# tbennun/capital

Hardware: NVIDIA H100
Metric: cholesky_tflops_fp64 (higher is better)
Workload: dtype f64

## Files before the change

capital_b200/csrc/api.cu:

```cuda
#include "common.cuh"
#include "dist.cuh"
#include "peer.cuh"
#include <math.h>
#include <stdlib.h>
#include <algorithm>

capital_status_t capital_ctx::workspace(const std::string& name, size_t bytes, void** out) {
  capital_ctx* ctx = this;
  DeviceBuf& b = pool[name];
  if (b.bytes < bytes) {
    if (b.p) CAP_CUDA(cudaFree(b.p));
    b.p = nullptr; b.bytes = 0;
    CAP_CUDA(cudaMalloc(&b.p, bytes));
    b.bytes = bytes;
    if (poison_workspace) {
      CAP_CUDA(cudaMemsetAsync(b.p, 0xFF, bytes, cudaStreamLegacy));
      CAP_CUDA(cudaStreamSynchronize(cudaStreamLegacy));
    }
  }
  *out = b.p;
  return CAPITAL_OK;
}

int capital_ctx::stream_id(cudaStream_t st) const {
// ... 368 lines not shown
capital_status_t capital_last_factor_ms(const capital_ctx* ctx_, float* ms) {
  capital_ctx* ctx = const_cast<capital_ctx*>(ctx_);
  if (!ctx || !ms) return CAPITAL_ERR_INVALID;
  CAP_CUDA(cudaEventElapsedTime(ms, ctx->ev_start, ctx->ev_stop));
  return CAPITAL_OK;
}

capital_status_t capital_timeline_begin(capital_ctx* ctx) {
  if (!ctx) return CAPITAL_ERR_INVALID;
  ctx->timeline = true; ctx->tl.clear(); ctx->tl_used = 0;
  return CAPITAL_OK;
}
capital_status_t capital_timeline_end(capital_ctx* ctx, double* out, int64_t cap_records, int64_t* n_records) {
  if (!ctx || !n_records) return CAPITAL_ERR_INVALID;
  ctx->timeline = false;
  CAP_CUDA(cudaSetDevice(ctx->device));
  CAP_CUDA(cudaDeviceSynchronize());
  *n_records = (int64_t)ctx->tl.size();
  if (out && !ctx->tl.empty()) {
    cudaEvent_t base = ctx->tl[0].e0;
    for (auto& r : ctx->tl) {
      float d = 0;
      if (cudaEventElapsedTime(&d, base, r.e0) == cudaSuccess && d < 0) base = r.e0;
    }
    for (int64_t i = 0; i < *n_records && i < cap_records; i++) {
      const auto& r = ctx->tl[i];
      float t0 = 0, t1 = 0;
      CAP_CUDA(cudaEventElapsedTime(&t0, base, r.e0));
      CAP_CUDA(cudaEventElapsedTime(&t1, base, r.e1));
      double* o = out + i * 8;
      o[0] = r.sid; o[1] = r.kind; o[2] = t0; o[3] = t1; o[4] = r.a; o[5] = r.b; o[6] = r.c; o[7] = 0;
    }
  }
  return CAPITAL_OK;
}
capital_status_t capital_probe_dmma_f64(capital_ctx* ctx, double* tflops, double* ms) {
  if (!ctx || !tflops || !ms) return CAPITAL_ERR_INVALID;
  CAP_CUDA(cudaSetDevice(ctx->device));
  return gemm_probe_dmma(ctx, tflops, ms);
}
capital_status_t capital_set_overlap(capital_ctx* ctx, int enabled) {
  if (!ctx) return CAPITAL_ERR_INVALID;
  ctx->no_overlap = !enabled;
  return CAPITAL_OK;
}
capital_status_t capital_profile_begin(capital_ctx* ctx) {
  if (!ctx) return CAPITAL_ERR_INVALID;
  ctx->profiling = true; ctx->prof_used = 0; ctx->prof_recs.clear();
  return CAPITAL_OK;
}
capital_status_t capital_profile_end(capital_ctx* ctx, double* kernel_ms, double* kernel_flops, int64_t* launches) {
  if (!ctx || !kernel_ms || !kernel_flops || !launches) return CAPITAL_ERR_INVALID;
  ctx->profiling = false;
  CAP_CUDA(cudaStreamSynchronize(ctx->stream));
  double ms = 0, fl = 0;
  for (auto& r : ctx->prof_recs) {
    float t = 0;
    CAP_CUDA(cudaEventElapsedTime(&t, r.e0, r.e1));
    ms += t; fl += r.flops;
  }
  *kernel_ms = ms; *kernel_flops = fl; *launches = (int64_t)ctx->prof_recs.size();
  ctx->prof_recs.clear(); ctx->prof_used = 0;
  return CAPITAL_OK;
}

capital_status_t capital_distribute_symmetric_f64(capital_ctx* ctx, double* A_local, int64_t n, int diag_dom) {
  if (!ctx || !A_local || n <= 0) return CAPITAL_ERR_INVALID;
  CAP_CUDA(cudaSetDevice(ctx->device));
  const int d = ctx->grid.d;
  const int64_t L = ceil_div(n, d);
  double* dev;
  CAP_TRY(cap_stage_out_begin(ctx, A_local, (size_t)L * L, "gen_out", &dev));
  CAP_TRY(gen_symmetric(ctx, ctx->stream, dev, L, L, L, n, ctx->grid.x, ctx->grid.y, d, diag_dom));
  CAP_TRY(cap_stage_out_end(ctx, A_local, (size_t)L * L, dev));
  CAP_CUDA(cudaStreamSynchronize(ctx->stream));
  return CAPITAL_OK;
}
capital_status_t capital_distribute_random_f64(capital_ctx* ctx, double* A_local, int64_t m, int64_t n, int64_t key) {
  if (!ctx || !A_local || n <= 0 || m <= 0) return CAPITAL_ERR_INVALID;
  CAP_CUDA(cudaSetDevice(ctx->device));
  const int c = ctx->grid.c, d = ctx->grid.d, x = ctx->grid.x, y = ctx->grid.y;
  const int64_t lr = ceil_div(m, d), lc = ceil_div(n, c);
  const int64_t pad_c = ((n % c != 0) && ((lc - 1) * c + x >= n)) ? lc - 1 : lc;
  const int64_t pad_r = ((m % d != 0) && ((lr - 1) * d + y >= m)) ? lr - 1 : lr;
  double* dev;
  CAP_TRY(cap_stage_out_begin(ctx, A_local, (size_t)lr * lc, "gen_out", &dev));
  CAP_TRY(gen_random(ctx, ctx->stream, dev, lr, lr, lc, pad_r, pad_c, key));
  CAP_TRY(cap_stage_out_end(ctx, A_local, (size_t)lr * lc, dev));
  CAP_CUDA(cudaStreamSynchronize(ctx->stream));
  return CAPITAL_OK;
}

capital_status_t capital_cholinv_factor_f64(capital_ctx* ctx, const double* A_local, int64_t n, const capital_cholinv_args_t* args,
                                            capital_structure_t ostruct, double* R_local, double* Rinv_local) {
  if (!ctx) return CAPITAL_ERR_INVALID;
  if (!A_local || !args || !R_local || !Rinv_local || n <= 0 || args->split <= 0 || args->dir != 'U') {
    ctx->set_error("cholinv::factor: invalid arguments (split > 0 and dir == 'U' are required, cholinv.hpp:9)");
    return CAPITAL_ERR_INVALID;
  }
  CAP_CUDA(cudaSetDevice(ctx->device));
  const capital_grid_t& g = ctx->grid;
  if (g.size > 1) return dist_cholinv_factor(ctx, A_local, n, args, ostruct, R_local, Rinv_local);

  const int64_t L = n, ld = round_up(L, 16);
  const size_t out_count = ostruct == CAPITAL_UPPERTRI_PACKED ? (size_t)L * (L + 1) / 2 : (size_t)L * L;
  cudaStream_t st = ctx->stream;
  ctx->io_used = 0;
  CAP_CUDA(cudaEventRecord(ctx->ev_start, st));
  double *W, *Rm, *Ri, *RiT, *dR, *dRinv;
  CAP_TRY(ctx->workspace("W", (size_t)ld * L * 8, (void**)&W));
  CAP_TRY(ctx->workspace("Rm", (size_t)ld * L * 8, (void**)&Rm));
  CAP_TRY(ctx->workspace("Ri", (size_t)ld * L * 8, (void**)&Ri));
  CAP_TRY(ctx->workspace("RiT", (size_t)ld * L * 8, (void**)&RiT));
  CAP_TRY(cap_stage_out_begin(ctx, R_local, out_count, "R_out", &dR));
  CAP_TRY(cap_stage_out_begin(ctx, Rinv_local, out_count, "Rinv_out", &dRinv));
  CAP_CUDA(cudaMemsetAsync(ctx->d_info, 0, sizeof(int), st));
  const int64_t bc = capital_cholinv_bc_dimension(L, g.c, g.d, args->bc_mult_dim);
  if (ostruct == CAPITAL_RECT) {
    CAP_CUDA(cudaMemsetAsync(Ri, 0, (size_t)ld * L * 8, st));
  } else {
    CAP_TRY(zero_band(ctx, st, L, Ri, ld));
    if (args->complete_inv == 0 && cholinv_node_splits(L, bc, (int)args->split)) {
      const int64_t s1 = L >> args->split;
      if (s1 > 0 && s1 < L) CAP_TRY(zero_block(ctx, st, s1, L - s1, Ri + s1 * ld, ld));
    }
  }
  CAP_TRY(zero_band(ctx, st, L, RiT, ld));
  if (ostruct == CAPITAL_RECT) CAP_CUDA(cudaMemsetAsync(Rm, 0, (size_t)ld * L * 8, st));

  HostIO io;
  io.ctx = ctx; io.L = L; io.ld = ld; io.Rm = Rm; io.Ri = Ri; io.dR = dR; io.dRinv = dRinv;
  io.hR = (dR != R_local) ? R_local : nullptr; io.hRinv = (dRinv != Rinv_local) ? Rinv_local : nullptr;
  io.packed = ostruct == CAPITAL_UPPERTRI_PACKED;
  io.rinv_streams = args->complete_inv == 0 && cholinv_node_splits(L, bc, (int)args->split);
  CholinvHooks hooks{&io, nullptr, nullptr};
  if (!cap_is_device_ptr(A_local)) {
    cudaEvent_t e0;
    CAP_TRY(io_event(ctx, &e0));
    CAP_CUDA(cudaEventRecord(e0, st));
    CAP_CUDA(cudaStreamWaitEvent(ctx->copy_in, e0, 0));
    const int64_t chunk = round_up(ceil_div(L, 16), 64);
    for (int64_t c0 = 0; c0 < L; c0 += chunk) {
      const int64_t nc = (c0 + chunk <= L) ? chunk : L - c0;
      const int64_t rows = c0 + nc;
      CAP_CUDA(cudaMemcpy2DAsync(W + c0 * ld, (size_t)ld * 8, A_local + c0 * L, (size_t)L * 8, (size_t)rows * 8, (size_t)nc,
                                 cudaMemcpyHostToDevice, ctx->copy_in));
      ctx->counters.h2d_bytes += rows * nc * 8;
      cudaEvent_t e;
      CAP_TRY(io_event(ctx, &e));
      CAP_CUDA(cudaEventRecord(e, ctx->copy_in));
      io.chunks.push_back({c0 + nc, e});
    }
    hooks.need_cols = hostio_need_cols;
  } else {
    CAP_TRY(copy_block(ctx, st, L, L, A_local, L, W, ld));
  }
  if (io.packed && L >= 2048) hooks.left_done = hostio_left_done;
  if (hooks.need_cols) hooks.cols_waited = hostio_cols_waited;
  if (hooks.left_done && (io.hR || io.hRinv)) {
    hooks.right_done = hostio_right_done;
    if (io.hRinv) hooks.inv_cols = hostio_inv_cols;
  }
  CAP_TRY(cholinv_local(ctx, st, L, W, ld, Rm, ld, Ri, ld, RiT, ld, args->complete_inv != 0, bc, (int)args->split, &hooks));
  if (ostruct == CAPITAL_UPPERTRI_PACKED) {
    {
      const int64_t c0 = io.cols_out;
      const size_t off = (size_t)c0 * (c0 + 1) / 2, cnt = out_count - off;
      CAP_TRY(pack_upper(ctx, st, L, Rm, ld, dR, 0, c0, L));
      if (io.hR && cnt) { CAP_CUDA(cudaMemcpyAsync(io.hR + off, dR + off, cnt * 8, cudaMemcpyDeviceToHost, st)); ctx->counters.d2h_bytes += (int64_t)cnt * 8; }
    }
    {
      const int64_t c0 = io.rinv_cols_out;
      const size_t off = (size_t)c0 * (c0 + 1) / 2, cnt = out_count - off;
      CAP_TRY(pack_upper(ctx, st, L, Ri, ld, dRinv, 0, c0, L));
      if (io.hRinv && cnt) { CAP_CUDA(cudaMemcpyAsync(io.hRinv + off, dRinv + off, cnt * 8, cudaMemcpyDeviceToHost, st)); ctx->counters.d2h_bytes += (int64_t)cnt * 8; }
    }
    if (io.e_out) CAP_CUDA(cudaStreamWaitEvent(st, io.e_out, 0));
  } else {
    CAP_TRY(triu_copy(ctx, st, L, Rm, ld, dR, L, 0));
    CAP_TRY(triu_copy(ctx, st, L, Ri, ld, dRinv, L, 0));
    CAP_TRY(cap_stage_out_end(ctx, R_local, out_count, dR));
    CAP_TRY(cap_stage_out_end(ctx, Rinv_local, out_count, dRinv));
  }
  CAP_CUDA(cudaEventRecord(ctx->ev_stop, st));
  return cap_check_info(ctx);
}

capital_status_t capital_cholinv_residual_f64(capital_ctx* ctx, const double* A_local, int64_t n, capital_structure_t structure,
                                              const double* R_local, double* residual) {
  if (!ctx || !A_local || !R_local || !residual || n <= 0) return CAPITAL_ERR_INVALID;
  CAP_CUDA(cudaSetDevice(ctx->device));
  const capital_grid_t& g = ctx->grid;
  if (g.size > 1) return dist_cholinv_residual(ctx, A_local, n, structure, R_local, residual);
  const int64_t L = n, ld = round_up(L, 16);
  cudaStream_t st = ctx->stream;
  const size_t r_count = structure == CAPITAL_UPPERTRI_PACKED ? (size_t)L * (L + 1) / 2 : (size_t)L * L;
  const double *dA, *dRin;
  CAP_TRY(cap_stage_in(ctx, A_local, (size_t)L * L, "A_in", &dA));
  CAP_TRY(cap_stage_in(ctx, R_local, r_count, "R_in", &dRin));
  double *E, *Rr;
  CAP_TRY(ctx->workspace("W", (size_t)ld * L * 8, (void**)&E));
  CAP_TRY(ctx->workspace("Rm", (size_t)ld * L * 8, (void**)&Rr));
  if (structure == CAPITAL_UPPERTRI_PACKED) CAP_TRY(unpack_upper(ctx, st, L, dRin, Rr, ld));
  else CAP_TRY(triu_copy(ctx, st, L, dRin, L, Rr, ld, 0));
  CAP_TRY(copy_block(ctx, st, L, L, dA, L, E, ld));
  CAP_CUDA(cudaMemsetAsync(ctx->d_scalars, 0, 2 * sizeof(double), st));
  CAP_TRY(sumsq_block(ctx, st, L, L, E, ld, 1, 0, 0, 1, ctx->d_scalars + 1));
  CAP_TRY(gemm_tn(ctx, st, L, L, L, 1.0, Rr, ld, Rr, ld, -1.0, E, ld,
                  CAPITAL_GEMM_A_UPPER | CAPITAL_GEMM_B_UPPER | CAPITAL_GEMM_C_UPPER));
  CAP_TRY(sumsq_block(ctx, st, L, L, E, ld, 1, 0, 0, 1, ctx->d_scalars));
  double h[2];
  CAP_CUDA(cudaMemcpyAsync(h, ctx->d_scalars, 2 * sizeof(double), cudaMemcpyDeviceToHost, st));
  CAP_CUDA(cudaStreamSynchronize(st));
  *residual = sqrt(h[0]) / sqrt(h[1]);
  return CAPITAL_OK;
}

static capital_status_t cholinv_solve_mode(capital_ctx* ctx, int64_t n, const capital_cholinv_args_t* args, capital_structure_t structure,
                                           const double* R_local, const double* Rinv_local, int64_t nrhs, const double* B, int64_t ldb,
                                           double* X, int64_t ldx, int mode, const char* what) {
  const bool apply_r = mode == SOLVE_R || mode == SOLVE_RT;
  if (!args || (apply_r ? !R_local : !Rinv_local) || !B || !X || n <= 0 || nrhs < 1 || ldb < n || ldx < n || args->split <= 0 ||
      args->dir != 'U' || (structure != CAPITAL_RECT && structure != CAPITAL_UPPERTRI_PACKED)) {
    ctx->set_error(std::string("cholinv::") + what + ": invalid arguments (" + (apply_r ? "R" : "Rinv") +
                   ", B, X non-null, nrhs >= 1, ldb, ldx >= n, split > 0 and dir == 'U')");
    return CAPITAL_ERR_INVALID;
  }
  CAP_CUDA(cudaSetDevice(ctx->device));
  const capital_grid_t& g = ctx->grid;
  if (g.size > 1) return dist_cholinv_solve(ctx, n, args, structure, R_local, Rinv_local, nrhs, B, ldb, X, ldx, mode);
  const int64_t L = n;
  const int64_t bc = capital_cholinv_bc_dimension(L, g.c, g.d, args->bc_mult_dim);
  const bool skipped = !apply_r && args->complete_inv == 0 && cholinv_node_splits(L, bc, (int)args->split);
  if (skipped && !R_local) {
    ctx->set_error(std::string("cholinv::") + what + ": the top-level Rinv12 block was skipped (complete_inv = 0), R is needed");
    return CAPITAL_ERR_INVALID;
  }
  const int64_t s1 = L >> args->split;
  const bool packed = structure == CAPITAL_UPPERTRI_PACKED;
  const size_t f_count = packed ? (size_t)L * (L + 1) / 2 : (size_t)L * L;
  const int64_t ldu = packed ? 0 : L;
  cudaStream_t st = ctx->stream;
  const double *dRi = nullptr, *dR = nullptr, *dB;
  if (!apply_r) CAP_TRY(cap_stage_in(ctx, Rinv_local, f_count, "solve_Rinv", &dRi));
  if (skipped || apply_r) CAP_TRY(cap_stage_in(ctx, R_local, f_count, "solve_R", &dR));
  CAP_TRY(cap_stage_in(ctx, B, (size_t)ldb * (nrhs - 1) + n, "solve_B", &dB));
  const bool x_host = !cap_is_device_ptr(X);
  double* dX = X;
  if (x_host) CAP_TRY(ctx->workspace("solve_X", (size_t)ldx * nrhs * 8, (void**)&dX));
  double *T, *T2;
  CAP_TRY(ctx->workspace("solve_T", (size_t)L * SOLVE_W * 8, (void**)&T));
  CAP_TRY(ctx->workspace("solve_T2", (size_t)L * SOLVE_W * 8, (void**)&T2));
  auto half_t = [&](const double* Bp, int64_t w) -> capital_status_t {
    if (!skipped) return tri_apply(ctx, st, {dRi, ldu, true, 0, L, 0, L, w, 1.0, Bp, 1, ldb, 0.0, nullptr, 0, T, 1, L});
    CAP_TRY(tri_apply(ctx, st, {dRi, ldu, true, 0, s1, 0, s1, w, 1.0, Bp, 1, ldb, 0.0, nullptr, 0, T, 1, L}));
    CAP_TRY(tri_apply(ctx, st, {dR, ldu, true, 0, s1, s1, L, w, -1.0, T, 1, L, 1.0, Bp, ldb, T2, 1, L}));
    return tri_apply(ctx, st, {dRi, ldu, true, s1, L, s1, L, w, 1.0, T2, 1, L, 0.0, nullptr, 0, T, 1, L});
  };
  auto half_n = [&](double* Xp, int64_t w) -> capital_status_t {
    if (!skipped) return tri_apply(ctx, st, {dRi, ldu, false, 0, L, 0, L, w, 1.0, T, 1, L, 0.0, nullptr, 0, Xp, 1, ldx});
    CAP_TRY(tri_apply(ctx, st, {dRi, ldu, false, s1, L, s1, L, w, 1.0, T, 1, L, 0.0, nullptr, 0, Xp, 1, ldx}));
    CAP_TRY(tri_apply(ctx, st, {dR, ldu, false, 0, s1, s1, L, w, -1.0, Xp, 1, ldx, 1.0, T, L, T2, 1, L}));
    return tri_apply(ctx, st, {dRi, ldu, false, 0, s1, 0, s1, w, 1.0, T2, 1, L, 0.0, nullptr, 0, Xp, 1, ldx});
  };
  for (int64_t p0 = 0; p0 < nrhs; p0 += SOLVE_W) {
    const int64_t w = std::min<int64_t>(SOLVE_W, nrhs - p0);
    const double* Bp = dB + p0 * ldb;
    double* Xp = dX + p0 * ldx;
    if (apply_r) {
      CAP_TRY(panel_add(ctx, st, L, w, Bp, ldb, nullptr, 0, T, L));
      CAP_TRY(tri_apply(ctx, st, {dR, ldu, mode == SOLVE_RT, 0, L, 0, L, w, 1.0, T, 1, L, 0.0, nullptr, 0, Xp, 1, ldx}));
      continue;
    }
    if (mode != SOLVE_RINV) CAP_TRY(half_t(Bp, w));
    else CAP_TRY(panel_add(ctx, st, L, w, Bp, ldb, nullptr, 0, T, L));
    if (mode != SOLVE_RINVT) CAP_TRY(half_n(Xp, w));
    else CAP_TRY(panel_add(ctx, st, L, w, T, L, nullptr, 0, Xp, ldx));
  }
  if (x_host) {
    CAP_CUDA(cudaMemcpy2DAsync(X, (size_t)ldx * 8, dX, (size_t)ldx * 8, (size_t)n * 8, (size_t)nrhs, cudaMemcpyDeviceToHost, st));
    ctx->counters.d2h_bytes += n * nrhs * 8;
    CAP_CUDA(cudaStreamSynchronize(st));
  }
  return CAPITAL_OK;
}

capital_status_t capital_cholinv_solve_f64(capital_ctx* ctx, int64_t n, const capital_cholinv_args_t* args, capital_structure_t structure,
                                           const double* R_local, const double* Rinv_local, int64_t nrhs, const double* B, int64_t ldb,
                                           double* X, int64_t ldx) {
  if (!ctx) return CAPITAL_ERR_INVALID;
  return cholinv_solve_mode(ctx, n, args, structure, R_local, Rinv_local, nrhs, B, ldb, X, ldx, SOLVE_FULL, "solve");
}

capital_status_t capital_cholinv_apply_rinv_f64(capital_ctx* ctx, int64_t n, const capital_cholinv_args_t* args, capital_structure_t structure,
                                                const double* R_local, const double* Rinv_local, int trans, int64_t nrhs, const double* B,
                                                int64_t ldb, double* X, int64_t ldx) {
  if (!ctx) return CAPITAL_ERR_INVALID;
  if (trans != 0 && trans != 1) {
    ctx->set_error("cholinv::apply_rinv: trans must be 0 (X = R^-1 B) or 1 (X = R^-T B)");
    return CAPITAL_ERR_INVALID;
  }
  return cholinv_solve_mode(ctx, n, args, structure, R_local, Rinv_local, nrhs, B, ldb, X, ldx, trans ? SOLVE_RINVT : SOLVE_RINV,
                            "apply_rinv");
}

capital_status_t capital_cholinv_apply_r_f64(capital_ctx* ctx, int64_t n, const capital_cholinv_args_t* args, capital_structure_t structure,
                                             const double* R_local, int trans, int64_t nrhs, const double* B, int64_t ldb, double* X,
                                             int64_t ldx) {
  if (!ctx) return CAPITAL_ERR_INVALID;
  if (trans != 0 && trans != 1) {
    ctx->set_error("cholinv::apply_r: trans must be 0 (X = R B) or 1 (X = R^T B)");
    return CAPITAL_ERR_INVALID;
  }
  return cholinv_solve_mode(ctx, n, args, structure, R_local, nullptr, nrhs, B, ldb, X, ldx, trans ? SOLVE_RT : SOLVE_R, "apply_r");
}

// ... 470 lines not shown
```

capital_b200/csrc/cholinv_local.cu:

```cuda
#include "common.cuh"

namespace {

int64_t split_point(int64_t n) {
  int64_t s1 = n >> 1;
  if (n > 2 * LEAF_MAX) s1 = round_up(s1, LEAF_MAX);
  else s1 = round_up(s1, 2);
  if (s1 >= n) s1 = n >> 1;
  return s1;
}

constexpr int64_t IN_CHUNK = 2048;

struct Rec {
  capital_ctx* ctx;
  cudaStream_t M;
  cudaStream_t S, D;
  cudaStream_t T;
  bool bands;
  double *W, *R, *Ri, *RiT;
  int64_t ldw, ldr, ldri, ldrit;
  int64_t bc;
  int split;
  const CholinvHooks* hooks;
// ... 21 lines not shown
}

struct Band {
  bool r12;
  int64_t o, s1, s2;
  cudaEvent_t wait;
  cudaStream_t st;
  int64_t edge = 0;
  cudaEvent_t done = nullptr;
};

capital_status_t issue_band(Rec& r, Band& b, int64_t split) {
  capital_ctx* ctx = r.ctx;
  const int64_t edge = split / 128 * 128;
  if (edge == 0) return CAPITAL_OK;
  cudaEvent_t e;
  CAP_TRY(new_event(ctx, &e));
  CAP_CUDA(cudaEventRecord(e, r.M));
  CAP_CUDA(cudaStreamWaitEvent(b.st, e, 0));
  if (b.wait) CAP_CUDA(cudaStreamWaitEvent(b.st, b.wait, 0));
  const int64_t o = b.o, s1 = b.s1, s2 = b.s2;
  const int64_t ldw = r.ldw, ldr = r.ldr, ldri = r.ldri, ldrit = r.ldrit;
  double* Ri = r.Ri + o * ldri + o;
  if (b.r12) {
    CAP_TRY(gemm_tn(ctx, b.st, edge, s2, edge, 1.0, Ri, ldri, r.W + (o + s1) * ldw + o, ldw, 0.0, r.R + (o + s1) * ldr + o, ldr,
                    CAPITAL_GEMM_A_UPPER));
  } else {
    double* Ri12 = Ri + s1 * ldri;
    CAP_TRY(gemm_tn(ctx, b.st, s1, edge, edge, -1.0, r.W + o * ldw + o + s1, ldw, Ri12 + s1, ldri, 0.0, Ri12, ldri, CAPITAL_GEMM_B_UPPER));
    CAP_TRY(transpose_block(ctx, b.st, s1, edge, Ri12, ldri, r.RiT + o * ldrit + o + s1, ldrit, 1.0));
  }
  CAP_TRY(new_event(ctx, &b.done));
  CAP_CUDA(cudaEventRecord(b.done, b.st));
  b.edge = edge;
  return CAPITAL_OK;
}

capital_status_t rec(Rec& r, int64_t o, int64_t n, bool complete, cudaEvent_t pending, cudaEvent_t pending22, int depth, Band* up) {
  capital_ctx* ctx = r.ctx;
  double* W = r.W + o * r.ldw + o;
  double* R = r.R + o * r.ldr + o;
  double* Ri = r.Ri + o * r.ldri + o;
  double* RiT = r.RiT + o * r.ldrit + o;
  const int64_t ldw = r.ldw, ldr = r.ldr, ldri = r.ldri, ldrit = r.ldrit;
  const int64_t s1 = choose_split(r, o, n, complete);
  if (s1 == 0) {
    if (r.hooks && r.hooks->need_cols) CAP_TRY(r.hooks->need_cols(r.hooks->user, r.M, o + n));
    if (pending22) CAP_CUDA(cudaStreamWaitEvent(r.M, pending22, 0));
    if (n <= LEAF_MAX) CAP_TRY(leaf_cholinv(ctx, r.M, (int)n, W, ldw, R, ldr, Ri, ldri, RiT, ldrit));
    else CAP_TRY(basecase_cholinv(ctx, r.M, (int)n, W, ldw, R, ldr, Ri, ldri, RiT, ldrit));
    return CAPITAL_OK;
  }
  const int64_t s2 = n - s1;
  double* W12 = W + s1 * ldw;
  double* W21 = W + s1;
  double* W22 = W + s1 * ldw + s1;
  double* R12 = R + s1 * ldr;
  double* Ri12 = Ri + s1 * ldri;
  double* Ri22 = Ri + s1 * ldri + s1;
  double* RiT21 = RiT + s1;

  cudaStream_t F = depth == 0 ? r.S : r.D;
  const bool bands = r.bands && s1 >= r.band_min;
  Band b12{true, o, s1, s2, pending, F};
  CAP_TRY(rec(r, o, s1, true, nullptr, nullptr, depth + 1, bands ? &b12 : nullptr));
  if (up) CAP_TRY(issue_band(r, *up, s1));
  if (depth <= 3 && o + n == r.total && r.hooks && r.hooks->left_done) CAP_TRY(r.hooks->left_done(r.hooks->user, r.M, o + s1, depth));
  const bool inflight = r.hooks && r.hooks->need_cols && r.hooks->cols_waited && r.hooks->cols_waited(r.hooks->user) < o + n;
  if (inflight && s2 >= 2 * IN_CHUNK) {
    if (pending) CAP_CUDA(cudaStreamWaitEvent(r.M, pending, 0));
    for (int64_t c0 = 0; c0 < s2;) {
      const int64_t nc = (s2 - c0 < IN_CHUNK + IN_CHUNK / 2) ? s2 - c0 : IN_CHUNK;
      CAP_TRY(r.hooks->need_cols(r.hooks->user, r.M, o + s1 + c0 + nc));
      CAP_TRY(gemm_tn(ctx, r.M, s1, nc, s1, 1.0, Ri, ldri, W12 + c0 * ldw, ldw, 0.0, R12 + c0 * ldr, ldr, CAPITAL_GEMM_A_UPPER));
      c0 += nc;
    }
  } else {
    if (r.hooks && r.hooks->need_cols) CAP_TRY(r.hooks->need_cols(r.hooks->user, r.M, o + n));
    if (pending) CAP_CUDA(cudaStreamWaitEvent(r.M, pending, 0));
    const int64_t e = b12.edge;
    CAP_TRY(gemm_tn_off(ctx, r.M, s1 - e, s2, s1, 1.0, Ri + e * ldri, ldri, W12, ldw, 0.0, R12 + e, ldr, CAPITAL_GEMM_A_UPPER, 0, (int)e));
    if (b12.done) CAP_CUDA(cudaStreamWaitEvent(r.M, b12.done, 0));
  }
  if (pending22) CAP_CUDA(cudaStreamWaitEvent(r.M, pending22, 0));
  cudaEvent_t e_r12 = nullptr, e_tt = nullptr, e_far12 = nullptr, e_far = nullptr;
  const bool use_side = r.S != nullptr && s1 >= r.ctx->side_min;
  if (use_side) {
    CAP_TRY(new_event(ctx, &e_r12));
    CAP_CUDA(cudaEventRecord(e_r12, r.M));
    CAP_CUDA(cudaStreamWaitEvent(F, e_r12, 0));
    if (complete) CAP_CUDA(cudaStreamWaitEvent(r.T, e_r12, 0));
  }
  cudaStream_t tS = use_side ? r.T : r.M;
  const int64_t h = choose_split(r, o + s1, s2, true);
  const int tf = trailing_uses_tf32(ctx, s1) ? ctx->trailing_mode : 0;
  if (use_side && h > 0 && s2 >= r.far_min) {
    if (tf) {
      CAP_TRY(gemm_tn_tf32(ctx, r.M, h, h, s1, -1.0, R12, ldr, R12, ldr, 1.0, W22, ldw, CAPITAL_GEMM_C_UPPER, tf));
      CAP_TRY(gemm_tn_tf32(ctx, F, h, s2 - h, s1, -1.0, R12, ldr, R12 + h * ldr, ldr, 1.0, W22 + h * ldw, ldw, 0, tf));
      CAP_TRY(new_event(ctx, &e_far12));
      CAP_CUDA(cudaEventRecord(e_far12, F));
      CAP_TRY(gemm_tn_tf32(ctx, F, s2 - h, s2 - h, s1, -1.0, R12 + h * ldr, ldr, R12 + h * ldr, ldr, 1.0, W22 + h * ldw + h, ldw,
                           CAPITAL_GEMM_C_UPPER, tf));
    } else {
      CAP_TRY(gemm_tn(ctx, r.M, h, h, s1, -1.0, R12, ldr, R12, ldr, 1.0, W22, ldw, CAPITAL_GEMM_C_UPPER));
      CAP_TRY(gemm_tn(ctx, F, h, s2 - h, s1, -1.0, R12, ldr, R12 + h * ldr, ldr, 1.0, W22 + h * ldw, ldw, 0));
      CAP_TRY(new_event(ctx, &e_far12));
      CAP_CUDA(cudaEventRecord(e_far12, F));
      CAP_TRY(gemm_tn(ctx, F, s2 - h, s2 - h, s1, -1.0, R12 + h * ldr, ldr, R12 + h * ldr, ldr, 1.0, W22 + h * ldw + h, ldw,
                      CAPITAL_GEMM_C_UPPER));
    }
    CAP_TRY(new_event(ctx, &e_far));
    CAP_CUDA(cudaEventRecord(e_far, F));
  } else if (tf) {
    CAP_TRY(gemm_tn_tf32(ctx, r.M, s2, s2, s1, -1.0, R12, ldr, R12, ldr, 1.0, W22, ldw, CAPITAL_GEMM_C_UPPER, tf));
  } else {
    CAP_TRY(gemm_tn(ctx, r.M, s2, s2, s1, -1.0, R12, ldr, R12, ldr, 1.0, W22, ldw, CAPITAL_GEMM_C_UPPER));
  }
  if (complete) {
    CAP_TRY(gemm_tn(ctx, tS, s2, s1, s1, 1.0, R12, ldr, RiT, ldrit, 0.0, W21, ldw, CAPITAL_GEMM_B_LOWER));
    if (use_side) {
      CAP_TRY(new_event(ctx, &e_tt));
      CAP_CUDA(cudaEventRecord(e_tt, r.T));
    }
  }
  const int64_t ct = s2 / 128;
  const bool inv_chunks = depth == 0 && r.hooks && r.hooks->inv_cols && ct >= 32;
  Band bi{false, o, s1, s2, e_tt, F};
  CAP_TRY(rec(r, o + s1, s2, true, e_far12, e_far, depth + 1, (bands && complete && !inv_chunks) ? &bi : nullptr));
  if (depth == 0 && r.hooks && r.hooks->right_done) CAP_TRY(r.hooks->right_done(r.hooks->user, r.M));
  if (complete) {
    if (e_tt) CAP_CUDA(cudaStreamWaitEvent(r.M, e_tt, 0));
    if (inv_chunks) {
      const int64_t e3 = ct - ct * 3 / 32, e2 = e3 - ct * 5 / 32, e1 = e2 - ct / 4;
      const int64_t edge[5] = {0, e1 * 128, e2 * 128, e3 * 128, s2};
      for (int i = 0; i < 4; i++) {
        const int64_t c0 = edge[i], c1 = edge[i + 1];
        if (c1 <= c0) continue;
        CAP_TRY(gemm_tn_off(ctx, r.M, s1, c1 - c0, c1, -1.0, W21, ldw, Ri22 + c0 * ldri, ldri, 0.0, Ri12 + c0 * ldri, ldri,
                            CAPITAL_GEMM_B_UPPER, (int)c0));
        CAP_TRY(r.hooks->inv_cols(r.hooks->user, r.M, o + s1 + c1));
      }
    } else {
      const int64_t c = bi.edge;
      CAP_TRY(gemm_tn_off(ctx, r.M, s1, s2 - c, s2, -1.0, W21, ldw, Ri22 + c * ldri, ldri, 0.0, Ri12 + c * ldri, ldri, CAPITAL_GEMM_B_UPPER,
                          (int)c));
    }
    CAP_TRY(transpose_block(ctx, r.M, s1, s2 - bi.edge, Ri12 + bi.edge * ldri, ldri, RiT21 + bi.edge, ldrit, 1.0));
    if (bi.done) CAP_CUDA(cudaStreamWaitEvent(r.M, bi.done, 0));
  }
  return CAPITAL_OK;
}

}

capital_status_t cholinv_local(capital_ctx* ctx, cudaStream_t st, int64_t n, double* W, int64_t ldw, double* R, int64_t ldr, double* Ri,
                               int64_t ldri, double* RiT, int64_t ldrit, bool complete_top, int64_t bc, int split,
                               const CholinvHooks* hooks, bool allow_side) {
  cudaStream_t M = (ctx->hi && allow_side) ? ctx->hi : st;
  cudaStream_t S = (allow_side && ctx->hi && ctx->side && n >= 1024 && !ctx->no_overlap) ? ctx->side : nullptr;
  cudaStream_t D = S ? ctx->side_deep[0] : nullptr, T = S ? ctx->side_deep[1] : nullptr;
  const bool bands = S && !(hooks && hooks->need_cols);
  ctx->dep_used = 0;
  cudaEvent_t e_in = nullptr, e_out = nullptr, e_s = nullptr;
  if (M != st) {
    CAP_TRY(new_event(ctx, &e_in));
    CAP_CUDA(cudaEventRecord(e_in, st));
    CAP_CUDA(cudaStreamWaitEvent(M, e_in, 0));
    if (S) CAP_CUDA(cudaStreamWaitEvent(S, e_in, 0));
  }
  const bool aligned = ((((uintptr_t)W | (uintptr_t)R | (uintptr_t)Ri | (uintptr_t)RiT) & 15) == 0) && !((ldw | ldr | ldri | ldrit) & 1);
  Rec r{ctx, M, S, D, T, bands, W, R, Ri, RiT, ldw, ldr, ldri, ldrit, bc, split, hooks, ctx->far_min, ctx->band_min, n, aligned};
  if (!cholinv_node_splits(n, bc, split)) complete_top = true;
  CAP_TRY(rec(r, 0, n, complete_top, nullptr, nullptr, 0, nullptr));
  if (M != st) {
    if (S) {
      for (cudaStream_t d : {S, D, T}) {
        CAP_TRY(new_event(ctx, &e_s));
        CAP_CUDA(cudaEventRecord(e_s, d));
        CAP_CUDA(cudaStreamWaitEvent(M, e_s, 0));
      }
    }
    CAP_TRY(new_event(ctx, &e_out));
    CAP_CUDA(cudaEventRecord(e_out, M));
    CAP_CUDA(cudaStreamWaitEvent(st, e_out, 0));
  }
  return CAPITAL_OK;
}
```

capital_b200/csrc/common.cuh:

```cuda
#pragma once
#include <cuda.h>
#include <cuda_runtime.h>
#include <stdint.h>
#include <stdio.h>
#include <stdlib.h>
#include <string.h>
#include <string>
#include <vector>
#include <map>
#include "../../include/capital_b200.h"

#define CAP_CUDA(call)                                                                                    \
  do {                                                                                                     \
    cudaError_t e__ = (call);                                                                              \
    if (e__ != cudaSuccess) {                                                                              \
      ctx->set_error(std::string(#call) + ": " + cudaGetErrorString(e__) + " (" + __FILE__ + ":" +         \
                     std::to_string(__LINE__) + ")");                                                      \
      return CAPITAL_ERR_CUDA;                                                                             \
    }                                                                                                      \
  } while (0)

#define CAP_TRY(call)                                  \
  do {                                                 \
    capital_status_t s__ = (call);                     \
// ... 36 lines not shown
  void* peer = nullptr;
  std::vector<cudaEvent_t> comm_pool;
  size_t comm_used = 0;
  std::string arena_signature;

  struct ProfRec { cudaEvent_t e0, e1; double flops; };
  bool profiling = false;
  int64_t far_min = 2048;
  int64_t side_min = 1024;
  int64_t band_min = 4096;
  bool no_overlap = false;
  bool poison_workspace = false;
  int trailing_mode = 0;
  bool tf32_ready = false;
  int64_t tf32_min_k = 256;
  int64_t tf32_launches = 0;
  double tf32_flops = 0.0;
  std::vector<cudaEvent_t> prof_pool;
  size_t prof_used = 0;
  std::vector<ProfRec> prof_recs;
  capital_status_t prof_event(cudaEvent_t* out) {
    if (prof_used == prof_pool.size()) {
      cudaEvent_t e;
      if (cudaEventCreate(&e) != cudaSuccess) { err = "cudaEventCreate failed"; return CAPITAL_ERR_CUDA; }
      prof_pool.push_back(e);
    }
    *out = prof_pool[prof_used++];
    return CAPITAL_OK;
  }

  struct TlRec { cudaEvent_t e0, e1; int sid, kind; double a, b, c; };
  bool timeline = false;
  std::vector<TlRec> tl;
  std::vector<cudaEvent_t> tl_pool;
  size_t tl_used = 0;
  int stream_id(cudaStream_t st) const;
  int tl_begin(cudaStream_t st, int kind, double a = 0, double b = 0, double c = 0);
  void tl_end(cudaStream_t st, int idx);

  void set_error(const std::string& s) { err = s; }
  capital_status_t workspace(const std::string& name, size_t bytes, void** out);
};

capital_status_t gemm_tn_init(capital_ctx* ctx);
capital_status_t leaf_init(capital_ctx* ctx);
capital_status_t gemm_probe_dmma(capital_ctx* ctx, double* tflops, double* ms);

constexpr int GEMM_NCLS_MAX = 2;
constexpr int GEMM_XPEERS_MAX = 3;
struct GemmXDev {
  int mode, c, z;
  double* Cpeer[GEMM_XPEERS_MAX];
};
struct GemmOperands {
  int ncls = 1;
  const double* A[GEMM_NCLS_MAX] = {nullptr, nullptr};
  const double* B[GEMM_NCLS_MAX] = {nullptr, nullptr};
  int64_t lda = 0, ldb = 0;
};
capital_status_t gemm_tn_x(capital_ctx* ctx, cudaStream_t st, int64_t m, int64_t n, int64_t k, double alpha, const GemmOperands& ops,
                           double beta, double* C, int64_t ldc, int flags, int noff, const GemmXDev* x, int moff = 0);
capital_status_t gemm_tn(capital_ctx* ctx, cudaStream_t st, int64_t m, int64_t n, int64_t k, double alpha, const double* A,
                         int64_t lda, const double* B, int64_t ldb, double beta, double* C, int64_t ldc, int flags);

capital_status_t gemm_tn_off(capital_ctx* ctx, cudaStream_t st, int64_t m, int64_t n, int64_t k, double alpha, const double* A,
                             int64_t lda, const double* B, int64_t ldb, double beta, double* C, int64_t ldc, int flags, int noff, int moff = 0);
capital_status_t gemm_tn_splitk(capital_ctx* ctx, cudaStream_t st, int64_t m, int64_t n, int64_t k, double alpha, const double* A,
                                int64_t lda, const double* B, int64_t ldb, double* C, int64_t ldc, int flags);
capital_status_t gemm_tn_t(capital_ctx* ctx, cudaStream_t st, int64_t m, int64_t n, int64_t k, double alpha, const double* A, int64_t lda,
                           const double* B, int64_t ldb, double* C, int64_t ldc, double* Ct, int64_t ldct, int flags);
int64_t gemm_splitk_chunks(const capital_ctx* ctx, int64_t m, int64_t n, int64_t k, int flags, bool* big);
struct GemmBatchOps {
  int64_t batch = 1;
  const double* A = nullptr;
  int64_t lda = 0, sa = 0;
  const double* B = nullptr;
  int64_t ldb = 0, sb = 0;
  int64_t sc = 0, sct = 0;
};
capital_status_t gemm_tn_batched(capital_ctx* ctx, cudaStream_t st, int64_t m, int64_t n, int64_t k, double alpha, const GemmBatchOps& b,
                                 double* C, int64_t ldc, double* Ct, int64_t ldct, int flags, bool gram);

capital_status_t gemm_tf32_init(capital_ctx* ctx);
capital_status_t gemm_tn_tf32(capital_ctx* ctx, cudaStream_t st, int64_t m, int64_t n, int64_t k, double alpha, const double* A, int64_t lda,
                              const double* B, int64_t ldb, double beta, double* C, int64_t ldc, int flags, int passes);
capital_status_t gemm_tn_tf32_x(capital_ctx* ctx, cudaStream_t st, int64_t m, int64_t n, int64_t k, double alpha, const GemmOperands& ops,
                                double beta, double* C, int64_t ldc, int flags, int noff, int passes);
static inline bool trailing_uses_tf32(const capital_ctx* ctx, int64_t k) { return ctx->trailing_mode != 0 && k >= ctx->tf32_min_k; }

capital_status_t transpose_block(capital_ctx* ctx, cudaStream_t st, int64_t rows, int64_t cols, const double* src,
                                 int64_t lds, double* dst, int64_t ldd, double scale);
capital_status_t copy_block(capital_ctx* ctx, cudaStream_t st, int64_t rows, int64_t cols, const double* src, int64_t lds,
                            double* dst, int64_t ldd);
capital_status_t zero_block(capital_ctx* ctx, cudaStream_t st, int64_t rows, int64_t cols, double* dst, int64_t ldd);
capital_status_t zero_band(capital_ctx* ctx, cudaStream_t st, int64_t n, double* a, int64_t ld);
capital_status_t pack_upper(capital_ctx* ctx, cudaStream_t st, int64_t n, const double* src, int64_t lds, double* packed,
                            int zero_diag, int64_t col_begin = 0, int64_t col_end = -1);
capital_status_t unpack_upper(capital_ctx* ctx, cudaStream_t st, int64_t n, const double* packed, double* dst, int64_t ldd);
capital_status_t triu_copy(capital_ctx* ctx, cudaStream_t st, int64_t n, const double* src, int64_t lds, double* dst,
                           int64_t ldd, int zero_diag);
capital_status_t sym_merge(capital_ctx* ctx, cudaStream_t st, int64_t n, const double* U, int64_t ldu, const double* S, int64_t lds,
                           bool s_trans, double* out, int64_t ldo, int x, int y, int d);
capital_status_t tril_half_copy(capital_ctx* ctx, cudaStream_t st, int64_t n, const double* src, int64_t lds, double* dst, int64_t ldd,
                                int x, int y, int d);
capital_status_t sym_pad_batched(capital_ctx* ctx, cudaStream_t st, int64_t n, int64_t nb, int64_t batch, const double* A, double* W);
capital_status_t triu_out_batched(capital_ctx* ctx, cudaStream_t st, int64_t n, int64_t batch, const double* src, int64_t lds, int64_t ss,
                                  double* dst);
capital_status_t gen_symmetric(capital_ctx* ctx, cudaStream_t st, double* A, int64_t ld, int64_t lrows, int64_t lcols,
                               int64_t n_global, int x, int y, int d, int diag_dom);
capital_status_t gen_random(capital_ctx* ctx, cudaStream_t st, double* A, int64_t ld, int64_t lrows, int64_t lcols,
                            int64_t pad_rows, int64_t pad_cols, int64_t key);
capital_status_t sumsq_block(capital_ctx* ctx, cudaStream_t st, int64_t rows, int64_t cols, const double* a, int64_t ld,
                             int upper_mode, int x, int y, int d, double* out);
capital_status_t sub_identity_local(capital_ctx* ctx, cudaStream_t st, int64_t n, double* a, int64_t ld);
capital_status_t gram_shift(capital_ctx* ctx, cudaStream_t st, int64_t n, double* G, int64_t ld, double coef);
capital_status_t gram_diag_partial(capital_ctx* ctx, cudaStream_t st, int64_t n, const double* G, int64_t ld, double* out);
capital_status_t gram_shift_by(capital_ctx* ctx, cudaStream_t st, int64_t n, double* G, int64_t ld, const double* parts, int nparts,
                               double coef);
capital_status_t gram_shift_batched(capital_ctx* ctx, cudaStream_t st, int64_t n, int64_t batch, double* G, int64_t ld, int64_t sg,
                                    double coef);
capital_status_t transpose_batched(capital_ctx* ctx, cudaStream_t st, int64_t rows, int64_t cols, int64_t batch, const double* src,
                                   int64_t lds, int64_t ss, double* dst, int64_t ldd, int64_t sd);

constexpr int LEAF_MAX = 64;
constexpr int BASECASE_MAX = 512;
struct BatchStrides { long long w = 0, r = 0, ri = 0, rit = 0; };
struct LeafBatch {
  int64_t batch;
  BatchStrides s;
  int* info;
  int cw;
};
capital_status_t basecase_cholinv(capital_ctx* ctx, cudaStream_t st, int nb, double* W, int64_t ldw, double* R, int64_t ldr,
                                  double* Ri, int64_t ldri, double* RiT, int64_t ldrit, const LeafBatch* bt = nullptr);
capital_status_t leaf_cholinv(capital_ctx* ctx, cudaStream_t st, int nb, const double* W, int64_t ldw, double* R, int64_t ldr,
                              double* Ri, int64_t ldri, double* RiT, int64_t ldrit, const LeafBatch* bt = nullptr);
static inline int batched_cluster_width(int64_t nb) {
  const char* e = getenv("CAPITAL_BATCHED_CW");
  if (e && atoi(e) == 8) return 8;
  const int64_t T = nb / 64;
  return T <= 2 ? 2 : T <= 4 ? 4 : 8;
}

struct CholinvHooks {
  void* user;
  capital_status_t (*need_cols)(void* user, cudaStream_t st, int64_t col_end);
  capital_status_t (*left_done)(void* user, cudaStream_t st, int64_t col_end, int depth);
  int64_t (*cols_waited)(void* user);
  capital_status_t (*right_done)(void* user, cudaStream_t st);
  capital_status_t (*inv_cols)(void* user, cudaStream_t st, int64_t col_end);
};
capital_status_t cholinv_local(capital_ctx* ctx, cudaStream_t st, int64_t n, double* W, int64_t ldw, double* R, int64_t ldr,
                               double* Ri, int64_t ldri, double* RiT, int64_t ldrit, bool complete_top, int64_t bc, int split,
                               const CholinvHooks* hooks = nullptr, bool allow_side = true);

constexpr int SOLVE_W = 32;
struct TriApply {
  const double* U;
  int64_t ldu;
  bool trans;
  int64_t r0, r1, c0, c1;
  int64_t nrhs;
  double alpha;
  const double* P;
  int64_t pinc, ldp;
  double beta;
  const double* Cin;
  int64_t ldcin;
  double* C;
  int64_t cinc, ldc;
  bool full = false;
  int64_t batch = 1, su = 0, sp = 0, scin = 0, sc = 0;
};
capital_status_t tri_apply(capital_ctx* ctx, cudaStream_t st, const TriApply& a);
capital_status_t tri_solve(capital_ctx* ctx, cudaStream_t st, const double* U, int64_t ldu, int64_t n, int64_t nrhs, double* Y,
                           int64_t ldy);
capital_status_t tri_solve_batched(capital_ctx* ctx, cudaStream_t st, const double* U, int64_t ldu, int64_t su, int64_t n, int64_t nrhs,
                                   double* Y, int64_t ldy, int64_t sy, int64_t batch);
capital_status_t panel_add(capital_ctx* ctx, cudaStream_t st, int64_t rows, int64_t w, const double* S, int64_t lds, const double* Cin,
                           int64_t ldcin, double* Out, int64_t ldo);

static inline int64_t round_up(int64_t a, int64_t b) { return (a + b - 1) / b * b; }
static inline bool cholinv_node_splits(int64_t n, int64_t bc, int split) { return n > bc && (n >> split) >= split && (n >> split) > 0; }
static inline int64_t ceil_div(int64_t a, int64_t b) { return (a + b - 1) / b; }
```

Baseline: 32.33.

## Overlap device input copy of right columns with left-half factorization

For device-resident input, the full copy of A into the workspace is replaced by a copy of only the upper-triangular columns. The left split's columns are copied on the main stream, while the right columns are copied on the copy_in stream, and an event is passed into the recursion so the right half waits only when it needs them. This hides the device-to-device copy behind the left-half factorization and moves less data, at the cost of extra events and depending on rec honouring the passed dependency events.

```diff
diff --git a/capital_b200/csrc/api.cu b/capital_b200/csrc/api.cu
--- a/capital_b200/csrc/api.cu
+++ b/capital_b200/csrc/api.cu
@@ -544,8 +544,6 @@
       io.chunks.push_back({c0 + nc, e});
     }
     hooks.need_cols = hostio_need_cols;
-  } else {
-    CAP_TRY(copy_block(ctx, st, L, L, A_local, L, W, ld));
   }
   if (io.packed && L >= 2048) hooks.left_done = hostio_left_done;
   if (hooks.need_cols) hooks.cols_waited = hostio_cols_waited;
@@ -553,7 +551,8 @@
     hooks.right_done = hostio_right_done;
     if (io.hRinv) hooks.inv_cols = hostio_inv_cols;
   }
-  CAP_TRY(cholinv_local(ctx, st, L, W, ld, Rm, ld, Ri, ld, RiT, ld, args->complete_inv != 0, bc, (int)args->split, &hooks));
+  const double* A_dev = hooks.need_cols ? nullptr : A_local;
+  CAP_TRY(cholinv_local(ctx, st, L, W, ld, Rm, ld, Ri, ld, RiT, ld, args->complete_inv != 0, bc, (int)args->split, &hooks, true, A_dev, L));
   if (ostruct == CAPITAL_UPPERTRI_PACKED) {
     {
       const int64_t c0 = io.cols_out;
diff --git a/capital_b200/csrc/cholinv_local.cu b/capital_b200/csrc/cholinv_local.cu
--- a/capital_b200/csrc/cholinv_local.cu
+++ b/capital_b200/csrc/cholinv_local.cu
@@ -197,27 +197,50 @@
   return CAPITAL_OK;
 }
 
+capital_status_t copy_upper_cols(capital_ctx* ctx, cudaStream_t st, const double* A, int64_t lda, double* W, int64_t ldw, int64_t c0, int64_t c1) {
+  constexpr int64_t CHUNK = 512;
+  for (int64_t c = c0; c < c1; c += CHUNK) {
+    const int64_t nc = std::min(CHUNK, c1 - c);
+    CAP_CUDA(cudaMemcpy2DAsync(W + c * ldw, (size_t)ldw * 8, A + c * lda, (size_t)lda * 8, (size_t)(c + nc) * 8, (size_t)nc,
+                               cudaMemcpyDeviceToDevice, st));
+  }
+  return CAPITAL_OK;
+}
+
 }
 
 capital_status_t cholinv_local(capital_ctx* ctx, cudaStream_t st, int64_t n, double* W, int64_t ldw, double* R, int64_t ldr, double* Ri,
                                int64_t ldri, double* RiT, int64_t ldrit, bool complete_top, int64_t bc, int split,
-                               const CholinvHooks* hooks, bool allow_side) {
+                               const CholinvHooks* hooks, bool allow_side, const double* A, int64_t lda) {
   cudaStream_t M = (ctx->hi && allow_side) ? ctx->hi : st;
   cudaStream_t S = (allow_side && ctx->hi && ctx->side && n >= 1024 && !ctx->no_overlap) ? ctx->side : nullptr;
   cudaStream_t D = S ? ctx->side_deep[0] : nullptr, T = S ? ctx->side_deep[1] : nullptr;
   const bool bands = S && !(hooks && hooks->need_cols);
   ctx->dep_used = 0;
-  cudaEvent_t e_in = nullptr, e_out = nullptr, e_s = nullptr;
+  cudaEvent_t e_in = nullptr, e_out = nullptr, e_s = nullptr, a_right = nullptr;
+  const bool aligned = ((((uintptr_t)W | (uintptr_t)R | (uintptr_t)Ri | (uintptr_t)RiT) & 15) == 0) && !((ldw | ldr | ldri | ldrit) & 1);
+  Rec r{ctx, M, S, D, T, bands, W, R, Ri, RiT, ldw, ldr, ldri, ldrit, bc, split, hooks, ctx->far_min, ctx->band_min, n, aligned};
+  if (!cholinv_node_splits(n, bc, split)) complete_top = true;
+  if (A) {
+    const int64_t s1 = S ? choose_split(r, 0, n, complete_top) : 0;
+    CAP_TRY(copy_upper_cols(ctx, st, A, lda, W, ldw, 0, s1 ? s1 : n));
+    if (s1) {
+      cudaEvent_t e;
+      CAP_TRY(new_event(ctx, &e));
+      CAP_CUDA(cudaEventRecord(e, st));
+      CAP_CUDA(cudaStreamWaitEvent(ctx->copy_in, e, 0));
+      CAP_TRY(copy_upper_cols(ctx, ctx->copy_in, A, lda, W, ldw, s1, n));
+      CAP_TRY(new_event(ctx, &a_right));
+      CAP_CUDA(cudaEventRecord(a_right, ctx->copy_in));
+    }
+  }
   if (M != st) {
     CAP_TRY(new_event(ctx, &e_in));
     CAP_CUDA(cudaEventRecord(e_in, st));
     CAP_CUDA(cudaStreamWaitEvent(M, e_in, 0));
     if (S) CAP_CUDA(cudaStreamWaitEvent(S, e_in, 0));
   }
-  const bool aligned = ((((uintptr_t)W | (uintptr_t)R | (uintptr_t)Ri | (uintptr_t)RiT) & 15) == 0) && !((ldw | ldr | ldri | ldrit) & 1);
-  Rec r{ctx, M, S, D, T, bands, W, R, Ri, RiT, ldw, ldr, ldri, ldrit, bc, split, hooks, ctx->far_min, ctx->band_min, n, aligned};
-  if (!cholinv_node_splits(n, bc, split)) complete_top = true;
-  CAP_TRY(rec(r, 0, n, complete_top, nullptr, nullptr, 0, nullptr));
+  CAP_TRY(rec(r, 0, n, complete_top, a_right, a_right, 0, nullptr));
   if (M != st) {
     if (S) {
       for (cudaStream_t d : {S, D, T}) {
diff --git a/capital_b200/csrc/common.cuh b/capital_b200/csrc/common.cuh
--- a/capital_b200/csrc/common.cuh
+++ b/capital_b200/csrc/common.cuh
@@ -212,7 +212,7 @@
 };
 capital_status_t cholinv_local(capital_ctx* ctx, cudaStream_t st, int64_t n, double* W, int64_t ldw, double* R, int64_t ldr,
                                double* Ri, int64_t ldri, double* RiT, int64_t ldrit, bool complete_top, int64_t bc, int split,
-                               const CholinvHooks* hooks = nullptr, bool allow_side = true);
+                               const CholinvHooks* hooks = nullptr, bool allow_side = true, const double* A = nullptr, int64_t lda = 0);
 
 constexpr int SOLVE_W = 32;
 struct TriApply {
```

Measured after the change: 32.81 (median of 6 runs). +1.5%, better.
